# UCL/gp_emulator

Hardware: AMD Instinct MI355X
Metric: test-points/sec for predict(mean+var+grad), N_train=250 D=11 (higher is better)
Workload: dtype f64

## Files before the change

gp_emulator_amd/csrc/gp_abi.hip:

```cpp
#include "gp_predict_hip.h"

#include <hip/hip_runtime.h>

#include <cctype>
#include <chrono>
#include <cmath>
#include <cstdarg>
#include <cstdio>
#include <cstdlib>
#include <cstring>
#include <exception>
#include <memory>
#include <atomic>
#include <mutex>
#include <new>
#include <thread>
#include <type_traits>
#include <vector>

#include <sched.h>

#include "gp_dispatch.hpp"
#include "gp_generic_kernel.hpp"
#include "gp_hessian_kernel.hpp"
// ... 64 lines not shown
    hipError_t e_ = (expr);                                                           \
    if (e_ != hipSuccess)                                                             \
      return fail(GP_ERR_HIP, "%s failed: %s (%s:%d)", #expr, hipGetErrorString(e_),  \
                  __FILE__, __LINE__);                                                \
  } while (0)

struct gp_model {
  int device;
  int dtype;
  int n_train, n_inputs;
  int kernel_d, kernel_nb;
  int kernel_nk;
  int n_emulators;
  long long xa_stride, frags_stride, sd_stride;
  void* d_xa;
  void* d_frags;
  void* d_sd;
  std::vector<double> scale_host, centre_host;
  std::vector<double> xs_host;
  std::mutex h_mutex;
  void* d_pfrags;
  long long pfrags_stride;
};

constexpr int kPipeSlotsMax = 6;
static int pipe_slots() {
  static const int n = [] {
    const char* ev = getenv("GP_HOST_SLOTS");
    const int v = ev ? atoi(ev) : 3;
    return v < 2 ? 2 : (v > kPipeSlotsMax ? kPipeSlotsMax : v);
  }();
  return n;
}
#define kPipeSlots pipe_slots()
struct gp_pipe {
  bool ready = false;
  hipStream_t stream[kPipeSlotsMax] = {};
  hipEvent_t done[kPipeSlotsMax] = {};
  hipStream_t up = nullptr, down = nullptr;
  hipEvent_t in_there[kPipeSlotsMax] = {}, computed[kPipeSlotsMax] = {};
  void* stage_in[kPipeSlotsMax] = {};
  void* stage_out[kPipeSlotsMax] = {};
  void* dev[kPipeSlotsMax] = {};

  size_t stage_in_bytes = 0, stage_out_bytes = 0, dev_bytes = 0;
  std::unique_ptr<gph::ThreadPool> pool;
};

struct gp_cached_model {
  gp_model* model = nullptr;
  int host_dtype = 0, compute_dtype = 0, n_train = 0, n_inputs = 0, theta_size = 0;
  bool with_invq = false;
  std::vector<char> key;
  unsigned long long stamp = 0;
};
constexpr int kModelCacheSlots = 4;

static const int kTicketSlots = 256;

struct gp_ctx {
  int device;
  hipStream_t stream;
  int compute_units;
  void* scratch;
  size_t scratch_bytes;
  void* dbg;
  unsigned* tickets = nullptr;
  std::atomic<unsigned> ticket_next{0};
  gp_pipe pipe;
  gp_cached_model cache[kModelCacheSlots];
  unsigned long long cache_clock = 0;
};

struct gp_event {
  int device;
  hipEvent_t ev;
};

static const int kKernelD[] = {
#define GP_V(d) d,
    GP_FOR_EACH_KERNEL_D(GP_V)
#undef GP_V
};
static const int kKernelNK[] = {
#define GP_V(d) d,
    GP_FOR_EACH_KERNEL_NK(GP_V)
#undef GP_V
};

static int pick_kernel(int n_train, int n_inputs, int* kd, int* knb, int* knk = nullptr) {
  *kd = *knb = -1;
  int nk = -1;
  for (int d : kKernelD)
    if (d >= n_inputs) { *kd = d; break; }
  static const bool whole_blocks = [] {
    const char* ev = getenv("GP_NO_KSKIP");
    return ev && atoi(ev) != 0;
  }();
  const int need = (n_train + 3) / 4;
  for (int k : kKernelNK)
    if (k >= need && !(whole_blocks && k % 4 != 0)) { nk = k; break; }
  if (nk > 0) *knb = (nk + 3) / 4;
  if (knk) *knk = nk;
  if (*kd > 0 && *knb > 0) return GP_OK;
  if (n_train <= gpk::gkMaxN && n_inputs <= gpk::gkMaxD) {
    if (*kd < 0) *kd = n_inputs;
    *knb = 0;
    if (knk) *knk = 0;
    return GP_OK;
  }
  return fail(GP_ERR_UNSUPPORTED,
              "shape outside the compiled kernel set: n_train=%d (max %d), n_inputs=%d (max %d)",
              n_train, gpk::gkMaxN, n_inputs, gpk::gkMaxD);
}
static inline int rows_padded(int n_train, int knb) { return knb > 0 ? 16 * knb : 16 * ((n_train + 15) / 16); }
static inline int row_stride_of(int kd) { return gpk::row_stride(kd); }

template <typename T, typename TH = T>
static int pack_model(const TH* expX, const TH* inputs, const TH* invQt, const TH* invQ, int N,
                      int D, int theta_size, T* xa, T* frags, T* sd, T* b) {
  if (!expX || !inputs || !invQt || !xa || !sd || !b || (invQ && !frags))
    return fail(GP_ERR_INVALID, "null pointer");
  if (N <= 0 || D <= 0) return fail(GP_ERR_INVALID, "n_train and n_inputs must be positive");
  if (theta_size < D + 1)
    return fail(GP_ERR_INVALID, "theta_size=%d < n_inputs+1=%d", theta_size, D + 1);
  int kd, knb;
  int rc = pick_kernel(N, D, &kd, &knb);
  if (rc) return rc;
  const int DS = row_stride_of(kd);
  const int NP = rows_padded(N, knb);
  std::vector<double> sdd(kd, 0.0), ctr(kd, 0.0);
  for (int d = 0; d < D; ++d) {
    sdd[d] = std::sqrt((double)expX[d]);
    double sum = 0.0;
    for (int i = 0; i < N; ++i) sum += (double)inputs[(size_t)i * D + d];
    ctr[d] = (double)(T)(sum / N);
  }
  for (int d = 0; d < kd; ++d) {
    sd[d] = (T)sdd[d];
    sd[kd + d] = (T)ctr[d];
  }
  *b = (T)expX[D];
  sd[2 * kd] = (T)expX[D];
  const double lnb = std::log((double)expX[D]);
  std::memset(xa, 0, sizeof(T) * (size_t)NP * DS);
  for (int i = 0; i < N; ++i) {
    const size_t row = (size_t)(knb > 0 ? gpk::point_slot<T>(i) : i) * DS;
    double n2 = 0.0;
    for (int d = 0; d < D; ++d) {
      const T xr = (T)((double)sd[d] * ((double)inputs[(size_t)i * D + d] - ctr[d]));
      xa[row + d] = xr;
      n2 += (double)xr * (double)xr;
    }
    xa[row + kd] = (T)invQt[i];
    xa[row + kd + 1] = (T)(lnb - 0.5 * n2);
  }
  if (!invQ) return GP_OK;
  if (knb == 0) {
    for (size_t q = 0; q < (size_t)N * N; ++q) frags[q] = (T)invQ[q];
    return GP_OK;
  }
  const int nfp = gpk::frag_count_padded(knb, gpk::Geo<T>::kChunk);
  std::memset(frags, 0, sizeof(T) * (size_t)nfp * 64);
  for (int J = 0; J < knb; ++J)
    for (int I = J; I < knb; ++I)
      for (int s = 0; s < 4; ++s) {
        T* f = frags + (size_t)gpk::frag_index(I, J, s, knb) * 64;
        for (int l = 0; l < 64; ++l) {
          const int i = gpk::slot_point<T>(gpk::own_index<T>(I, s, l >> 4));
          const int j = gpk::slot_point<T>(16 * J + (l & 15));
          if (i >= N || j >= N) continue;
          double v = (double)invQ[(size_t)i * N + j];
          if (I > J) v += (double)invQ[(size_t)j * N + i];
          f[l] = (T)v;
        }
      }
  return GP_OK;
}

template <typename T>
static hipError_t launch(int knk, int kd, const gpk::PredictArgs<T>& a, int grid, bool var, hipStream_t s);
template <>
hipError_t launch<float>(int knk, int kd, const gpk::PredictArgs<float>& a, int grid, bool var, hipStream_t s) {
  switch (knk) {
#define GP_CASE(nk) \
  case nk: return var ? gpk::launch_predict_f32_##nk(kd, a, grid, s) : gpk::launch_mean_grad_f32_##nk(kd, a, grid, s);
    GP_FOR_EACH_KERNEL_NK(GP_CASE)
#undef GP_CASE
  }
  return hipErrorInvalidValue;
}
template <>
hipError_t launch<double>(int knk, int kd, const gpk::PredictArgs<double>& a, int grid, bool var, hipStream_t s) {
  switch (knk) {
#define GP_CASE(nk) \
  case nk: return var ? gpk::launch_predict_f64_##nk(kd, a, grid, s) : gpk::launch_mean_grad_f64_##nk(kd, a, grid, s);
    GP_FOR_EACH_KERNEL_NK(GP_CASE)
#undef GP_CASE
  }
  return hipErrorInvalidValue;
}

extern "C" {

const char* gp_last_error_string(void) { return g_err; }
const char* gp_version_string(void) { return "gp_predict_hip 0.1 (gfx950)"; }

int gp_device_count(int* count) {
  if (!count) return fail(GP_ERR_INVALID, "null pointer");
  int n = 0;
  hipError_t e = hipGetDeviceCount(&n);
  if (e != hipSuccess) {
    *count = 0;
    return fail(GP_ERR_NO_DEVICE, "hipGetDeviceCount: %s", hipGetErrorString(e));
  }
  *count = n;
  return GP_OK;
}

int gp_ctx_create(int device, gp_ctx** out) {
  if (!out) return fail(GP_ERR_INVALID, "null pointer");
  *out = nullptr;
  int n = 0;
  int rc = gp_device_count(&n);
  if (rc) return rc;
  if (n <= 0) return fail(GP_ERR_NO_DEVICE, "no HIP device visible");
  if (device < 0 || device >= n) return fail(GP_ERR_INVALID, "device %d out of range [0,%d)", device, n);
  HIP_TRY(hipSetDevice(device));
  hipDeviceProp_t prop;
  HIP_TRY(hipGetDeviceProperties(&prop, device));
  gp_ctx* c = new (std::nothrow) gp_ctx();
  if (!c) return fail(GP_ERR_NOMEM, "out of host memory");
  c->device = device;
  c->compute_units = prop.multiProcessorCount;
  c->scratch = nullptr;
  c->scratch_bytes = 0;
  c->dbg = nullptr;
  hipError_t e = hipStreamCreateWithFlags(&c->stream, hipStreamNonBlocking);
  if (e != hipSuccess) {
    delete c;
    return fail(GP_ERR_HIP, "hipStreamCreate: %s", hipGetErrorString(e));
  }
  e = hipMalloc((void**)&c->tickets, 4 * kTicketSlots * sizeof(unsigned));
  if (e == hipSuccess) e = hipMemset(c->tickets, 0, 4 * kTicketSlots * sizeof(unsigned));
  if (e != hipSuccess) {
    if (c->tickets) (void)hipFree(c->tickets);
    (void)hipStreamDestroy(c->stream);
    delete c;
    return fail(GP_ERR_HIP, "context item counters: %s", hipGetErrorString(e));
  }
  *out = c;
  return GP_OK;
}

int gp_ctx_destroy(gp_ctx* ctx) {
  if (!ctx) return GP_OK;
  (void)hipSetDevice(ctx->device);
  (void)hipStreamSynchronize(ctx->stream);
  for (auto& c : ctx->cache)
    if (c.model) gp_model_destroy(c.model);
  if (ctx->scratch) (void)hipFree(ctx->scratch);
  if (ctx->tickets) (void)hipFree(ctx->tickets);
  gp_pipe& pp = ctx->pipe;
  pp.pool.reset();
  for (int k = 0; k < kPipeSlots; ++k) {
    if (pp.stream[k]) (void)hipStreamSynchronize(pp.stream[k]);
    if (pp.stage_in[k]) (void)hipHostFree(pp.stage_in[k]);
    if (pp.stage_out[k]) (void)hipHostFree(pp.stage_out[k]);
    if (pp.dev[k]) (void)hipFree(pp.dev[k]);
    if (pp.done[k]) (void)hipEventDestroy(pp.done[k]);
    if (pp.in_there[k]) (void)hipEventDestroy(pp.in_there[k]);
    if (pp.computed[k]) (void)hipEventDestroy(pp.computed[k]);
    if (pp.stream[k]) (void)hipStreamDestroy(pp.stream[k]);
  }
  if (pp.up) { (void)hipStreamSynchronize(pp.up); (void)hipStreamDestroy(pp.up); }
  if (pp.down) { (void)hipStreamSynchronize(pp.down); (void)hipStreamDestroy(pp.down); }
  (void)hipStreamDestroy(ctx->stream);
  delete ctx;
  return GP_OK;
}

int gp_ctx_set_debug_buffer(gp_ctx* ctx, void* d_buffer) {
  if (!ctx) return fail(GP_ERR_INVALID, "null context");
  ctx->dbg = d_buffer;
  return GP_OK;
}

int gp_ctx_synchronize(gp_ctx* ctx) {
  if (!ctx) return fail(GP_ERR_INVALID, "null context");
  HIP_TRY(hipSetDevice(ctx->device));
  HIP_TRY(hipStreamSynchronize(ctx->stream));
  return GP_OK;
}

int gp_ctx_device_info(gp_ctx* ctx, int* compute_units, int64_t* hbm_bytes, char* name, int name_len) {
  if (!ctx) return fail(GP_ERR_INVALID, "null context");
  hipDeviceProp_t prop;
  HIP_TRY(hipGetDeviceProperties(&prop, ctx->device));
  if (compute_units) *compute_units = prop.multiProcessorCount;
  if (hbm_bytes) *hbm_bytes = (int64_t)prop.totalGlobalMem;
  if (name && name_len > 0) {
    snprintf(name, name_len, "%s (%s)", prop.name, prop.gcnArchName);
  }
  return GP_OK;
}

// ... 1780 lines not shown
```

gp_emulator_amd/csrc/gp_generic_kernel.hpp:

```cpp
#pragma once
#include "gp_predict_kernel.hpp"

namespace gpk {

constexpr int gkThreads = 256;
constexpr int gkMaxN = 1024;
constexpr int gkMaxD = 64;

template <typename T>
struct GenericArgs {
  const T* xa;
  const T* invQ;
  const T* sd;
  const T* testing;
  T* mu;
  T* var;
  T* deriv;
  long long M;
  int N, D;
  int ds, acol, dk;
  int deriv_row_major;
  int want_var;
};

template <typename T>
__device__ inline T row16_sum(T v) {
  v += __shfl_xor(v, 8, 64);
  v += __shfl_xor(v, 4, 64);
  v += __shfl_xor(v, 2, 64);
  v += __shfl_xor(v, 1, 64);
  return v;
}

template <typename T>
__global__ __launch_bounds__(gkThreads) void predict_generic_kernel(GenericArgs<T> p) {
  typedef Real<T> R;
  extern __shared__ __attribute__((aligned(16))) unsigned char g_raw[];
  T* s_k = reinterpret_cast<T*>(g_raw);
  const int ns = p.N + 1;
  T* s_t = s_k + 16 * ns;

  const int tid = threadIdx.x;
  const int ml = tid >> 4;
  const int jl = tid & 15;
  const T b = p.sd[2 * p.dk];
  const long long n_tiles = (p.M + 15) / 16;

  for (long long tile = blockIdx.x; tile < n_tiles; tile += gridDim.x) {
    const long long m = tile * 16 + ml;
    const long long mc = m < p.M ? m : p.M - 1;
    __syncthreads();
    for (int d = jl; d < p.D; d += 16)
      s_t[ml * p.D + d] = p.sd[d] * (p.testing[mc * p.D + d] - p.sd[p.dk + d]);
    __syncthreads();

    const T* t = &s_t[ml * p.D];
    T mu = T(0);
    for (int i = jl; i < p.N; i += 16) {
      const T* row = &p.xa[(long long)i * p.ds];
      T r2 = T(0);
      for (int d = 0; d < p.D; ++d) {
        const T dl = row[d] - t[d];
        r2 = fma(dl, dl, r2);
      }
      const T k = b * R::exp_(T(-0.5) * r2);
      s_k[ml * ns + i] = k;
      mu = fma(k, row[p.acol], mu);
    }
    mu = row16_sum(mu);
    if (jl == 0 && m < p.M) p.mu[m] = mu;

    for (int d = 0; d < p.D; ++d) {
      T gsum = T(0);
      for (int i = jl; i < p.N; i += 16) {
        const T* row = &p.xa[(long long)i * p.ds];
        gsum = fma(s_k[ml * ns + i] * row[p.acol], row[d] - t[d], gsum);
      }
      gsum = row16_sum(gsum) * p.sd[d];
      if (jl == 0 && m < p.M) {
        if (p.deriv_row_major) p.deriv[m * p.D + d] = gsum;
        else p.deriv[(long long)d * p.M + m] = gsum;
      }
    }
    if (!p.want_var) continue;
    __syncthreads();

    const T* kr = &s_k[ml * ns];
    T acc = T(0);
    for (int j = jl; j < p.N; j += 16) {
      T s = T(0);
      for (int i = 0; i < p.N; ++i) s = fma(p.invQ[(long long)i * p.N + j], kr[i], s);
      acc = fma(s, kr[j], acc);
    }
    acc = row16_sum(acc);
    if (jl == 0 && m < p.M) p.var[m] = b - acc;
  }
}

}
```

gp_emulator_amd/csrc/gp_hessian_kernel.hpp:

```cpp
#pragma once
#include "gp_predict_kernel.hpp"

#ifndef GP_HESS_ABLATE
#define GP_HESS_ABLATE 0
#endif

namespace gpk {

template <typename T>
struct HessianArgs {
  const T* xa;
  const T* sd;
  const T* testing;
  T* hess;
  long long M;
  int d_actual;
  int nb;
  int n_emulators;
  long long xa_stride, sd_stride, hess_stride;
};

constexpr int hkWaves = 4;
constexpr int hkThreads = hkWaves * 64;
constexpr int hkRowsPerWG = hkWaves * kTile;

__host__ __device__ constexpr int pairs_in_rows(int D, int lo, int hi) {
  int n = 0;
  for (int d = lo; d < hi; ++d) n += D - d;
  return n;
}
__host__ __device__ constexpr int split_row(int D) {
  int best = 0, bestdiff = 1 << 30;
  for (int r = 0; r <= D; ++r) {
    int a = pairs_in_rows(D, 0, r), b = pairs_in_rows(D, r, D);
    int diff = a > b ? a - b : b - a;
    if (diff < bestdiff) { bestdiff = diff; best = r; }
  }
  return best;
}

template <typename T, int D, int LO, int HI>
__device__ __forceinline__ void hessian_pass(const T* s_xa, const T* s_sd, const T (&t)[D], T b,
                                             int nb, int g, bool row_ok, int d_actual, T* out) {
  typedef Real<T> R;
  constexpr int DS = row_stride(D);
  constexpr int NP_ = pairs_in_rows(D, LO, HI);
  T acc[NP_];
#pragma unroll
  for (int q = 0; q < NP_; ++q) acc[q] = T(0);
  T mu = T(0);
  T nxt[D + 1];
  {
    const T* row = &s_xa[R::own_sub(0, g) * DS];
#pragma unroll
    for (int d = 0; d <= D; ++d) nxt[d] = row[d];
  }
#pragma unroll 1
  for (int qq = 0; qq < 4 * nb; ++qq) {
    T dl[D];
    T r2p[4] = {T(0), T(0), T(0), T(0)};
#pragma unroll
    for (int d = 0; d < D; ++d) {
      dl[d] = nxt[d] - t[d];
      r2p[d & 3] = fma(dl[d], dl[d], r2p[d & 3]);
    }
    const T alpha = nxt[D];
    {
      const int qn = (qq + 1 < 4 * nb) ? qq + 1 : 0;
      const T* row = &s_xa[(16 * (qn >> 2) + R::own_sub(qn & 3, g)) * DS];
#pragma unroll
      for (int d = 0; d <= D; ++d) nxt[d] = row[d];
    }
    const T r2 = (r2p[0] + r2p[1]) + (r2p[2] + r2p[3]);
    const T w = b * R::exp_(T(-0.5) * r2) * alpha;
    mu += w;
    int q = 0;
#pragma unroll
    for (int d = LO; d < HI; ++d) {
      const T wd = w * dl[d];
#pragma unroll
      for (int d2 = d; d2 < D; ++d2) {
        acc[q] = fma(wd, dl[d2], acc[q]);
        ++q;
      }
    }
  }
#if GP_HESS_ABLATE == 2
  T keep = mu;
#pragma unroll
  for (int q = 0; q < NP_; ++q) keep += acc[q];
  if (keep == T(-12345.678)) out[0] = keep;
  return;
#endif
  mu = xor_reduce_groups(mu);
  int q = 0;
#pragma unroll
  for (int d = LO; d < HI; ++d) {
#pragma unroll
    for (int d2 = d; d2 < D; ++d2) {
      T v = xor_reduce_groups(acc[q]) * (s_sd[d] * s_sd[d2]);
      if (d2 == d) v = fma(-(s_sd[d] * s_sd[d]), mu, v);
      ++q;
#if GP_HESS_ABLATE == 1
      if (v == T(-12345.678)) out[0] = v;
#else
      if (row_ok && d < d_actual && d2 < d_actual) {
        if ((d & 3) == g) out[d * d_actual + d2] = v;
        if (d2 != d && (d2 & 3) == g) out[d2 * d_actual + d] = v;
      }
#endif
    }
  }
}

template <typename T, int D, bool BATCH = false>
__global__ __launch_bounds__(hkThreads, 2) void hessian_kernel(HessianArgs<T> p) {
  typedef Real<T> R;
  constexpr int DS = row_stride(D);
  constexpr int NPAIR = D * (D + 1) / 2;
  constexpr int kSplit = (NPAIR * (int)sizeof(T) / 4 > 144) ? split_row(D) : 0;
  extern __shared__ __attribute__((aligned(16))) unsigned char s_raw[];
  T* s_xa = reinterpret_cast<T*>(s_raw);

  const int tid = threadIdx.x;
  const int lane = tid & 63;
  const int wave = __builtin_amdgcn_readfirstlane(tid >> 6);
  const int ml = lane & 15;
  const int g = lane >> 4;
  const int np = 16 * p.nb;

  T* s_sd = s_xa + np * DS;
  const long long n_groups = (p.M + hkRowsPerWG - 1) / hkRowsPerWG;
  const long long n_items = BATCH ? n_groups * p.n_emulators : n_groups;
  T b;
  auto load_emulator = [&](int e_) __attribute__((always_inline)) {
    const T* xa_ = p.xa;
    const T* sd_ = p.sd;
    if constexpr (BATCH) {
      xa_ += (long long)e_ * p.xa_stride;
      sd_ += (long long)e_ * p.sd_stride;
    }
    for (int i = tid; i < np * DS; i += hkThreads) s_xa[i] = xa_[i];
    if (tid < 2 * D) s_sd[tid] = ((tid % D) < p.d_actual) ? sd_[tid] : T(0);
    b = sd_[2 * D];
  };
  int cur_e = BATCH ? (int)(blockIdx.x / n_groups) : 0;
  load_emulator(cur_e);
  __syncthreads();

  for (long long item = blockIdx.x; item < n_items; item += gridDim.x) {
    long long grp = item;
    T* hess_e = p.hess;
    if constexpr (BATCH) {
      const int e = (int)(item / n_groups);
      grp = item - e * n_groups;
      hess_e += (long long)e * p.hess_stride;
      if (e != cur_e) {
        cur_e = e;
        __syncthreads();
        load_emulator(e);
        __syncthreads();
      }
    }
    const long long m = grp * hkRowsPerWG + wave * kTile + ml;
    const long long mc = m < p.M ? m : p.M - 1;
    T t[D];
#pragma unroll
    for (int d = 0; d < D; ++d)
      t[d] = (d < p.d_actual) ? s_sd[d] * (p.testing[mc * p.d_actual + d] - s_sd[D + d]) : T(0);
    T* out = hess_e + mc * (long long)p.d_actual * p.d_actual;
    const bool row_ok = m < p.M;
    if constexpr (kSplit > 0) {
      hessian_pass<T, D, 0, kSplit>(s_xa, s_sd, t, b, p.nb, g, row_ok, p.d_actual, out);
      hessian_pass<T, D, kSplit, D>(s_xa, s_sd, t, b, p.nb, g, row_ok, p.d_actual, out);
    } else {
      hessian_pass<T, D, 0, D>(s_xa, s_sd, t, b, p.nb, g, row_ok, p.d_actual, out);
    }
  }
}

}
```

gp_emulator_amd/csrc/gp_predict_few_kernel.hpp:

```cpp
#pragma once
#include "gp_predict_kernel.hpp"

namespace gpk {

constexpr int fkWaves = 8;
constexpr int fkThreads = fkWaves * 64;
constexpr int fkMaxKSteps = 4 * 20;

template <typename T, int D, bool kVar = true>
__global__ __launch_bounds__(fkThreads, 2) void predict_few_kernel(PredictArgs<T> p, int NB) {
  typedef Real<T> R;
  typedef typename R::acc_t acc_t;
  constexpr int DS = row_stride(D);
  constexpr int kVals = D + 2;

  __shared__ __attribute__((aligned(16))) T s_xa[4 * fkMaxKSteps * row_stride(D)];
  __shared__ T s_k[kVar ? fkMaxKSteps : 1][64];
  __shared__ T s_part[fkWaves][kTile][kVals];

  const int tid = threadIdx.x;
  const int lane = tid & 63;
  const int w = __builtin_amdgcn_readfirstlane(tid >> 6);
  const int ml = lane & 15, g = lane >> 4;
  const int n_tiles = (int)((p.M + kTile - 1) / kTile);
  const int e = blockIdx.x / n_tiles, tile = blockIdx.x - e * n_tiles;
  const int NKS = 4 * NB;

  const T* xa = p.xa + e * p.xa_stride;
  const T* frags = p.frags + e * p.frags_stride;
  (void)frags;
  const T* sdp = p.sd + e * p.sd_stride;
  const long long m = (long long)tile * kTile + ml;
  const long long mc = m < p.M ? m : p.M - 1;

  {
    const int n = 16 * NB * DS;
#pragma unroll 4
    for (int i = tid; i < n; i += fkThreads) s_xa[i] = xa[i];
  }

  T t[D];
  T gm = T(0);
#pragma unroll
  for (int d = 0; d < D; ++d) {
    const bool live = d < p.d_actual;
    const int dc = live ? d : p.d_actual - 1;
    const T sc = !live ? T(0) : p.rows_prescaled ? T(1) : sdp[d];
    const T ce = (!live || p.rows_prescaled) ? T(0) : sdp[D + d];
    t[d] = sc * (p.testing[mc * p.d_actual + dc] - ce);
    gm = fma(t[d], t[d], gm);
  }
  gm *= T(-0.5);
  const T poison = gm - gm;
  const T b = sdp[2 * D];
  __syncthreads();

  T mu = T(0);
  T ga[D];
#pragma unroll
  for (int d = 0; d < D; ++d) ga[d] = T(0);
#pragma unroll 1
  for (int ks = w; ks < NKS; ks += fkWaves) {
    const int i = own_index<T>(ks >> 2, ks & 3, g);
    const T* row = &s_xa[i * DS];
    T x[D];
#pragma unroll
    for (int d = 0; d < D; ++d) x[d] = row[d];
    const T al = row[D];
    T k;
    if constexpr (R::kExpand) {
      k = row[D + 1] + gm;
#pragma unroll
      for (int d = 0; d < D; ++d) k = fma(x[d], t[d], k);
      k = R::exp_(k);
    } else {
      T r2 = T(0);
#pragma unroll
      for (int d = 0; d < D; ++d) {
        x[d] -= t[d];
        r2 = fma(x[d], x[d], r2);
      }
      k = b * R::exp_(T(-0.5) * r2);
    }
    if constexpr (kVar) s_k[ks][lane] = k;
    const T wgt = k * al;
    mu += wgt;
#pragma unroll
    for (int d = 0; d < D; ++d) ga[d] = fma(wgt, x[d], ga[d]);
  }
  mu = xor_reduce_groups(mu);
  xor_reduce_groups_n<T, D>(ga);
  if (g == 0) {
    s_part[w][ml][0] = mu;
#pragma unroll
    for (int d = 0; d < D; ++d) s_part[w][ml][1 + d] = ga[d];
  }
  __syncthreads();

  if constexpr (kVar) {
  T vacc = T(0);
  auto column_block = [&](const int J) __attribute__((always_inline)) {
    const T* f = frags + ((size_t)frag_index(J, J, 0, NB) * 64 + lane);
    const int n = 4 * (NB - J);
    acc_t acc = acc_t{T(0), T(0), T(0), T(0)};
    T a_cur[4], a_nxt[4];
#pragma unroll
    for (int s = 0; s < 4; ++s) a_cur[s] = f[(size_t)s * 64];
#pragma unroll 1
    for (int q = 0; q < n; q += 4) {
      const int qn = q + 4 < n ? q + 4 : q;
#pragma unroll
      for (int s = 0; s < 4; ++s) a_nxt[s] = f[(size_t)(qn + s) * 64];
#pragma unroll
      for (int s = 0; s < 4; ++s) acc = R::mfma(a_cur[s], s_k[4 * J + q + s][lane], acc);
#pragma unroll
      for (int s = 0; s < 4; ++s) a_cur[s] = a_nxt[s];
    }
#pragma unroll
    for (int r = 0; r < 4; ++r) vacc = fma(acc[r], s_k[4 * J + r][lane], vacc);
  };
  for (int pr = w; 2 * pr < NB; pr += fkWaves) {
    column_block(pr);
    if (NB - 1 - pr != pr) column_block(NB - 1 - pr);
  }
  vacc = xor_reduce_groups(vacc);
  if (g == 0) s_part[w][ml][1 + D] = vacc;
  __syncthreads();
  }

  if (w == 0 && m < p.M) {
    auto total = [&](const int v) __attribute__((always_inline)) {
      T s = s_part[0][ml][v];
#pragma unroll
      for (int k = 1; k < fkWaves; ++k) s += s_part[k][ml][v];
      return s;
    };
    const T mean = total(0) + poison;
    T* o_mu = p.mu + e * p.M;
    T* o_der = p.deriv + e * p.M * p.d_actual;
    if (g == 0) o_mu[m] = mean;
    if constexpr (kVar) {
      if (g == 1) p.var[e * p.M + m] = b - total(1 + D) + poison;
    }
#pragma unroll
    for (int d = 0; d < D; ++d) {
      if ((d & 3) == g && d < p.d_actual) {
        const T gsum = total(1 + d);
        const T gd = sdp[d] * (R::kExpand ? fma(-t[d], mean, gsum) : gsum + poison);
        if (p.deriv_row_major) o_der[m * p.d_actual + d] = gd;
        else o_der[(long long)d * p.M + m] = gd;
      }
    }
  }
}

}
```

gp_emulator_amd/csrc/gp_predict_kernel.hpp:

```cpp
#pragma once
#include <hip/hip_runtime.h>
#include <stdint.h>
#include <type_traits>
#include <utility>

namespace gpk {

#ifndef GP_WAVES
#define GP_WAVES 8
#endif
#ifndef GP_WAVES_F32
#define GP_WAVES_F32 12
#endif
#ifndef GP_CHUNK
#define GP_CHUNK 64
#endif
#ifndef GP_CHUNK_F32
#define GP_CHUNK_F32 192
#endif
#ifndef GP_ABLATE
#define GP_ABLATE 0
#endif
#ifndef GP_AHEAD
#define GP_AHEAD 4
#endif
#ifndef GP_AHEAD_F32
#define GP_AHEAD_F32 8
#endif
#ifndef GP_RING_PIN
#define GP_RING_PIN 1
#endif
#ifndef GP_MU_DOUBLE
#define GP_MU_DOUBLE 1
#endif
#ifndef GP_ESTRIN
#define GP_ESTRIN 0
#endif
#ifndef GP_DOTSPLIT
#define GP_DOTSPLIT 1
#endif
#ifndef GP_GROUP_F64
#define GP_GROUP_F64 1
#endif
#ifndef GP_STAMPS
#define GP_STAMPS 0
#endif
constexpr int kTile = 16;
template <typename T, bool kVar = true> struct Geo {
  static constexpr int kWaves = sizeof(T) == 8 ? GP_WAVES : GP_WAVES_F32;
  static constexpr int kThreads = kWaves * 64;
#ifndef GP_WG_PER_CU_SMALL
#define GP_WG_PER_CU_SMALL 0
#endif
  static constexpr int kWGPerCU = kWaves >= 8 ? 1 : (GP_WG_PER_CU_SMALL > 0 ? GP_WG_PER_CU_SMALL : 8 / kWaves);
  static constexpr int kWavesPerSimd = kWaves >= 8 ? kWaves / 4 : kWGPerCU * kWaves / 4;
  static constexpr int kRowsPerWG = kWaves * kTile;
  static constexpr int kChunk = sizeof(T) == 8 ? GP_CHUNK : GP_CHUNK_F32;
};
#ifndef GP_MG_WAVES
#define GP_MG_WAVES 12
#endif
#ifndef GP_MG_WAVES_F32
#define GP_MG_WAVES_F32 16
#endif
#ifndef GP_MG_WG_PER_CU
#define GP_MG_WG_PER_CU 1
#endif
template <typename T> struct Geo<T, false> {
  static constexpr int kWaves = sizeof(T) == 8 ? GP_MG_WAVES : GP_MG_WAVES_F32;
  static constexpr int kThreads = kWaves * 64;
  static constexpr int kWGPerCU = GP_MG_WG_PER_CU;
  static constexpr int kWavesPerSimd = kWGPerCU * kWaves / 4;
  static constexpr int kRowsPerWG = kWaves * kTile;
  static constexpr int kChunk = 1;
};

typedef double f64x4 __attribute__((ext_vector_type(4)));
typedef float f32x4 __attribute__((ext_vector_type(4)));

template <typename F, int... Is>
__device__ __forceinline__ void static_for_impl(F&& f, std::integer_sequence<int, Is...>) {
  (f(std::integral_constant<int, Is>{}), ...);
}
template <int N, typename F>
__device__ __forceinline__ void static_for(F&& f) {
  static_for_impl(f, std::make_integer_sequence<int, N>{});
}

template <typename T> struct Real;
template <> struct Real<double> {
  typedef f64x4 acc_t;
  static constexpr bool kExpand = true;
  static constexpr int kGroup = GP_GROUP_F64;
  __host__ __device__ static constexpr int own_sub(int r, int g) { return 4 * r + g; }
  __device__ static inline acc_t mfma(double a, double b, acc_t c) {
    return __builtin_amdgcn_mfma_f64_16x16x4f64(a, b, c, 0, 0, 0);
  }
  __device__ static inline double exp_(double x) {
    x = __builtin_fmax(x, -1000.0);
    const double n = __builtin_rint(x * 1.4426950408889634);
    double r = fma(n, -6.93147180559945286e-01, x);
    r = fma(n, -2.31904681384629956e-17, r);
#if GP_ESTRIN
    const double r2 = r * r;
    const double p01 = fma(1.00000000000000666e+00, r, 1.0);
    const double p23 = fma(1.66666666665544028e-01, r, 5.00000000000000555e-01);
    const double p45 = fma(8.33333338566834801e-03, r, 4.16666666665732183e-02);
    const double p67 = fma(1.98411702695461072e-04, r, 1.38888889324666632e-03);
    const double p89 = fma(2.76401812311866076e-06, r, 2.48015043709117912e-05);
    const double r4 = r2 * r2;
    const double q0 = fma(r2, p23, p01);
    const double q1 = fma(r2, p67, p45);
    const double q2 = fma(r2, 2.76263485910095559e-07, p89);
    const double r8 = r4 * r4;
    const double s0 = fma(r4, q1, q0);
    const double p = fma(r8, q2, s0);
#else
    double p = 2.76263485910095559e-07;
    p = fma(p, r, 2.76401812311866076e-06);
    p = fma(p, r, 2.48015043709117912e-05);
    p = fma(p, r, 1.98411702695461072e-04);
    p = fma(p, r, 1.38888889324666632e-03);
    p = fma(p, r, 8.33333338566834801e-03);
    p = fma(p, r, 4.16666666665732183e-02);
    p = fma(p, r, 1.66666666665544028e-01);
    p = fma(p, r, 5.00000000000000555e-01);
    p = fma(p, r, 1.00000000000000666e+00);
    p = fma(p, r, 1.0);
#endif
    return ldexp(p, (int)n);
  }
  template <int GP>
  __device__ static inline void exp_n(double (&x)[GP]) {
    double n[GP], r[GP], p[GP];
#pragma unroll
    for (int u = 0; u < GP; ++u) x[u] = __builtin_fmax(x[u], -1000.0);
#pragma unroll
    for (int u = 0; u < GP; ++u) n[u] = __builtin_rint(x[u] * 1.4426950408889634);
#pragma unroll
    for (int u = 0; u < GP; ++u) r[u] = fma(n[u], -6.93147180559945286e-01, x[u]);
#pragma unroll
    for (int u = 0; u < GP; ++u) r[u] = fma(n[u], -2.31904681384629956e-17, r[u]);
#pragma unroll
    for (int u = 0; u < GP; ++u) p[u] = 2.76263485910095559e-07;
    constexpr double c[10] = {2.76401812311866076e-06, 2.48015043709117912e-05, 1.98411702695461072e-04,
                              1.38888889324666632e-03, 8.33333338566834801e-03, 4.16666666665732183e-02,
                              1.66666666665544028e-01, 5.00000000000000555e-01, 1.00000000000000666e+00, 1.0};
#pragma unroll
    for (int j = 0; j < 10; ++j) {
#pragma unroll
      for (int u = 0; u < GP; ++u) p[u] = fma(p[u], r[u], c[j]);
    }
#pragma unroll
    for (int u = 0; u < GP; ++u) x[u] = ldexp(p[u], (int)n[u]);
  }
};
template <> struct Real<float> {
  typedef f32x4 acc_t;
  static constexpr bool kExpand = false;
#ifndef GP_GROUP_F32
#define GP_GROUP_F32 2
#endif
  static constexpr int kGroup = GP_GROUP_F32;
  __host__ __device__ static constexpr int own_sub(int r, int g) { return 4 * g + r; }
  __device__ static inline acc_t mfma(float a, float b, acc_t c) {
    return __builtin_amdgcn_mfma_f32_16x16x4f32(a, b, c, 0, 0, 0);
  }
  __device__ static inline float exp_(float x) { return __expf(x); }
  template <int GP>
  __device__ static inline void exp_n(float (&x)[GP]) {
#pragma unroll
    for (int u = 0; u < GP; ++u) x[u] = __expf(x[u]);
  }
};

template <typename T>
__host__ __device__ constexpr int own_index(int I, int s, int g) {
  return 16 * I + Real<T>::own_sub(s, g);
}

template <typename T>
__host__ __device__ constexpr int point_slot(int n) {
  return 16 * (n / 16) + Real<T>::own_sub((n % 16) / 4, n % 4);
}
template <typename T>
__host__ __device__ constexpr int slot_point(int slot) {
  for (int q = 0; q < 16; ++q)
    if (Real<T>::own_sub(q / 4, q % 4) == slot % 16) return 16 * (slot / 16) + q;
  return -1;
}

struct FragId { int I, J, s; };
__host__ __device__ constexpr int frag_count(int NB) { return NB * (NB + 1) / 2 * 4; }
__host__ __device__ constexpr int frag_col_offset(int J, int NB) { return J * NB - J * (J - 1) / 2; }
__host__ __device__ constexpr FragId frag_at(int n, int NB) {
  const int pair = n >> 2;
  int J = 0;
  while (J + 1 < NB && frag_col_offset(J + 1, NB) <= pair) ++J;
  return FragId{J + pair - frag_col_offset(J, NB), J, n & 3};
}
__host__ __device__ constexpr int frag_index(int I, int J, int s, int NB) {
  return (frag_col_offset(J, NB) + (I - J)) * 4 + s;
}
__host__ __device__ constexpr int frag_count_padded(int NB, int chunk) {
  return (frag_count(NB) + chunk - 1) / chunk * chunk;
}

__host__ __device__ constexpr int row_stride(int D) { return (D + 2 + 3) & ~3; }
#ifndef GP_XA_PAD
#define GP_XA_PAD 1
#endif
template <typename T> __host__ __device__ constexpr int xa_lds_stride(int D) {
  return (GP_XA_PAD && sizeof(T) == 4 && row_stride(D) % 16 == 0) ? row_stride(D) + 4 : row_stride(D);
}

#ifndef GP_FRAG_BUFS
#define GP_FRAG_BUFS 3
#endif
#ifndef GP_FRAG_BUFS_F32
#define GP_FRAG_BUFS_F32 2
#endif
constexpr int kLdsBudget = 160 * 1024;
constexpr int kLdsSlack = 32;
template <typename T>
__host__ __device__ constexpr int predict_lds_bytes(int D, int NK, int bufs) {
  const int NP = 16 * ((NK + 3) / 4);
  return (int)sizeof(T) * (NP * xa_lds_stride<T>(D) + bufs * Geo<T>::kChunk * 64 + (2 * D + 1) + 2 * D +
                           2 * Geo<T>::kWaves * kTile * D) + kLdsSlack;
}
template <typename T>
__host__ __device__ constexpr int frag_buffers(int D, int NK) {
  const int want = sizeof(T) == 8 ? GP_FRAG_BUFS : GP_FRAG_BUFS_F32;
  return want > 2 && predict_lds_bytes<T>(D, NK, want) <= kLdsBudget ? want : 2;
}

template <typename T>
struct PredictArgs {
  const T* xa;
  const T* frags;
  const T* sd;
  const T* testing;
  T* mu;
  T* var;
  T* deriv;
  long long M;
  int d_actual;
  int deriv_row_major;
  int n_emulators;
  long long xa_stride, frags_stride, sd_stride;
  unsigned long long* dbg;
  int rows_prescaled;
};

template <int XOR>
__device__ __forceinline__ unsigned swap_halves(unsigned x, unsigned& other) {
  if constexpr (XOR == 16) {
    auto r = __builtin_amdgcn_permlane16_swap(x, x, false, false);
    other = r[1];
    return r[0];
  } else {
    auto r = __builtin_amdgcn_permlane32_swap(x, x, false, false);
    other = r[1];
    return r[0];
  }
}
template <int XOR>
__device__ __forceinline__ float pair_sum(float v) {
  unsigned o, a = swap_halves<XOR>(__float_as_uint(v), o);
  return __uint_as_float(a) + __uint_as_float(o);
}
template <int XOR>
__device__ __forceinline__ double pair_sum(double v) {
  const unsigned long long u = (unsigned long long)__double_as_longlong(v);
  unsigned lo_o, hi_o;
  const unsigned lo_a = swap_halves<XOR>((unsigned)u, lo_o);
  const unsigned hi_a = swap_halves<XOR>((unsigned)(u >> 32), hi_o);
  const double a = __longlong_as_double((long long)(((unsigned long long)hi_a << 32) | lo_a));
  const double o = __longlong_as_double((long long)(((unsigned long long)hi_o << 32) | lo_o));
  return a + o;
}

template <typename T, int N>
__device__ inline void xor_reduce_groups_n(T* v) {
#pragma unroll
  for (int i = 0; i < N; ++i) v[i] = pair_sum<32>(pair_sum<16>(v[i]));
}

template <typename T>
__device__ inline T xor_reduce_groups(T v) {
  return pair_sum<32>(pair_sum<16>(v));
}

template <typename T, int kWaves = Geo<T>::kWaves, int kChunk = Geo<T>::kChunk>
__device__ __forceinline__ void stage_chunk(const T* src, T* dst, int wave, int lane) {
  constexpr int kBytes = kChunk * 64 * (int)sizeof(T);
  constexpr int kPieces = kBytes / 1024;
  static_assert(kPieces * 1024 == kBytes, "chunk must be whole 1 KiB pieces");
  const unsigned voff = (unsigned)lane * 16u;
  const unsigned lds0 = (unsigned)(uintptr_t)(
      (__attribute__((address_space(3))) char*)(reinterpret_cast<char*>(dst)));
#pragma unroll
  for (int pc0 = 0; pc0 < kPieces; pc0 += kWaves) {
    const int pc = pc0 + wave;
    if (pc0 + kWaves <= kPieces || pc < kPieces) {
      const char* s = reinterpret_cast<const char*>(src) + pc * 1024;
      const unsigned m0v = __builtin_amdgcn_readfirstlane(lds0 + pc * 1024);
      unsigned keep;
      asm volatile(
          "s_mov_b32 %0, m0\n\t"
          "s_mov_b32 m0, %1\n\t"
          "s_nop 4\n\t"
          "global_load_lds_dwordx4 %2, %3\n\t"
          "s_mov_b32 m0, %0"
          : "=&s"(keep)
          : "s"(m0v), "v"(voff), "s"(s)
          : "memory");
    }
  }
}
template <typename T, int NP>
__device__ __forceinline__ void stage_pieces(const T* src, T* dst, int first_piece, int lane) {
  const unsigned voff = (unsigned)lane * 16u;
  const unsigned lds0 = (unsigned)(uintptr_t)(
      (__attribute__((address_space(3))) char*)(reinterpret_cast<char*>(dst)));
#pragma unroll
  for (int i = 0; i < NP; ++i) {
    const int pc = first_piece + i;
    const char* s = reinterpret_cast<const char*>(src) + pc * 1024;
    const unsigned m0v = __builtin_amdgcn_readfirstlane(lds0 + pc * 1024);
    unsigned keep;
    asm volatile(
        "s_mov_b32 %0, m0\n\t"
        "s_mov_b32 m0, %1\n\t"
        "s_nop 4\n\t"
        "global_load_lds_dwordx4 %2, %3\n\t"
        "s_mov_b32 m0, %0"
        : "=&s"(keep)
        : "s"(m0v), "v"(voff), "s"(s)
        : "memory");
  }
}
__device__ __forceinline__ void dma_wait() { asm volatile("s_waitcnt vmcnt(0)" ::: "memory"); }

#if GP_STAMPS == 1
#define GP_STAMP(seg)                                                                    \
  do {                                                                                   \
    __builtin_amdgcn_sched_barrier(0);                                                   \
    unsigned long long now_;                                                             \
    asm volatile("s_memtime %0\n\ts_waitcnt lgkmcnt(0)" : "=s"(now_)::"memory");         \
    __builtin_amdgcn_sched_barrier(0);                                                   \
    seg_sum[seg] += now_ - seg_t0;                                                       \
    seg_t0 = now_;                                                                       \
  } while (0)
#else
#define GP_STAMP(seg) do { } while (0)
#endif

template <typename T, int D, int NK, bool kVar = true>
__global__ __launch_bounds__((Geo<T, kVar>::kThreads), (Geo<T, kVar>::kWavesPerSimd)) void predict_kernel(PredictArgs<T> p) {
  typedef Real<T> R;
  typedef Geo<T, kVar> G;
  constexpr int kThreads = G::kThreads;
  constexpr int kRowsPerWG = G::kRowsPerWG;
  typedef typename R::acc_t acc_t;
  constexpr int NB = (NK + 3) / 4;
  constexpr int KL = NK - 4 * (NB - 1);
  constexpr int NP = 16 * NB;
  constexpr int DSG = row_stride(D);
  constexpr int DS = xa_lds_stride<T>(D);
  constexpr int NF = frag_count(NB);
  constexpr int kChunk = G::kChunk;
  constexpr int NCH = (NF + kChunk - 1) / kChunk;
  constexpr int kBufs = kVar ? frag_buffers<T>(D, NK) : 1;
  constexpr int kLook = kBufs - 2;

  __shared__ __attribute__((aligned(16))) T s_xa[NP * DS];
  __shared__ __attribute__((aligned(16))) T s_fr[kBufs][kVar ? kChunk * 64 : 1];
  __shared__ T s_sd[2 * D + 1];
  __shared__ T s_ts[2 * D];
  __shared__ T s_rows[2][G::kWaves][kTile * D];
  static_assert(!kVar || (int)(sizeof(s_xa) + sizeof(s_fr) + sizeof(s_sd) + sizeof(s_ts) + sizeof(s_rows)) + kLdsSlack ==
                             predict_lds_bytes<T>(D, NK, kBufs), "predict_lds_bytes() does not count the kernel's LDS arrays");

  const int tid = threadIdx.x;
  const int lane = tid & 63;
  const int wave = __builtin_amdgcn_readfirstlane(tid >> 6);
  const int ml = lane & 15;
  const int g = lane >> 4;

  const int n_groups = (int)((p.M + kRowsPerWG - 1) / kRowsPerWG);
  int e = 0, cur_e = -1;
  int grp = blockIdx.x;
  while (grp >= n_groups && e < p.n_emulators) { grp -= n_groups; ++e; }

  constexpr int NJ = (kTile * D + 63) / 64;
  auto fetch_rows = [&](int grp_, T (&regs)[NJ]) {
    const long long e0 = ((long long)grp_ * kRowsPerWG + wave * kTile) * p.d_actual;
    const long long emax = p.M * p.d_actual - 1;
#pragma unroll
    for (int j = 0; j < NJ; ++j) {
      long long e_ = e0 + lane + 64 * j;
      e_ = e_ < emax ? e_ : emax;
      regs[j] = p.testing[e_];
    }
  };
  auto stash_rows = [&](int buf_, const T (&regs)[NJ]) {
#pragma unroll
    for (int j = 0; j < NJ; ++j) asm volatile("" ::"v"(regs[j]));
#pragma unroll
    for (int j = 0; j < NJ; ++j)
      if (lane + 64 * j < kTile * p.d_actual) s_rows[buf_][wave][lane + 64 * j] = regs[j];
  };
  int rbuf = 0;
  T rregs[NJ];
  if (e < p.n_emulators) {
    fetch_rows(grp, rregs);
    stash_rows(0, rregs);
  }
#if GP_STAMPS
  unsigned long long seg_sum[8] = {0, 0, 0, 0, 0, 0, 0, 0};
  unsigned long long seg_t0;
  asm volatile("s_memtime %0\n\ts_waitcnt lgkmcnt(0)" : "=s"(seg_t0)::"memory");
#endif

  for (; e < p.n_emulators;) {
    if (e != cur_e) {
      cur_e = e;
      __syncthreads();
      const T* xa = p.xa + e * p.xa_stride;
      for (int i = tid; i < NP * DSG; i += kThreads) s_xa[(i / DSG) * DS + i % DSG] = xa[i];
      const T* sdp = p.sd + e * p.sd_stride;
      if (tid < 2 * D + 1) {
        const bool live = tid == 2 * D || (tid % D) < p.d_actual;
        s_sd[tid] = live ? sdp[tid] : T(0);
        if (tid < 2 * D)
          s_ts[tid] = !live ? T(0) : !p.rows_prescaled ? sdp[tid] : tid < D ? T(1) : T(0);
      }
      if constexpr (!kVar) __syncthreads();
    }
    const T* frags = p.frags + e * p.frags_stride;
    T* o_mu = p.mu + e * p.M;
    T* o_der = p.deriv + e * p.M * p.d_actual;
    const long long m = (long long)grp * kRowsPerWG + wave * kTile + ml;
    const long long mc = m < p.M ? m : p.M - 1;

    if constexpr (kVar) {
      __syncthreads();
      static_for<1 + kLook>([&](auto cc) {
        constexpr int c = decltype(cc)::value;
        if constexpr (c < NCH) stage_chunk<T, G::kWaves, kChunk>(frags + c * kChunk * 64, &s_fr[c][0], wave, lane);
      });
    } else {
      (void)frags;
      __builtin_amdgcn_fence(__ATOMIC_ACQ_REL, "wavefront");
      __builtin_amdgcn_wave_barrier();
    }
    const T b = s_sd[2 * D];
    GP_STAMP(0);

    T t[D];
    T gm = T(0);
    {
      T sdv[D], cv[D], rv[D];
#pragma unroll
      for (int d = 0; d < D; ++d) {
        const int dc = d < p.d_actual ? d : p.d_actual - 1;
        sdv[d] = s_ts[d];
        cv[d] = s_ts[D + d];
        rv[d] = s_rows[rbuf][wave][ml * p.d_actual + dc];
      }
#pragma unroll
      for (int d = 0; d < D; ++d) {
        t[d] = sdv[d] * (rv[d] - cv[d]);
        gm = fma(t[d], t[d], gm);
      }
    }
    gm *= T(-0.5);
    const T poison = gm - gm;

    asm volatile("" :: "v"(gm));
    int e_next = e, grp_next = grp + gridDim.x;
    while (grp_next >= n_groups && e_next < p.n_emulators) { grp_next -= n_groups; ++e_next; }
    fetch_rows(e_next < p.n_emulators ? grp_next : grp, rregs);

    GP_STAMP(1);
    T kv[NK];
#if GP_MU_DOUBLE
    double mu = 0.0;
#else
    T mu = T(0);
#endif
    T ga[D];
#pragma unroll
    for (int d = 0; d < D; ++d) ga[d] = T(0);

    constexpr int GP = R::kGroup;
    static_for<(NK + GP - 1) / GP>([&](auto qc) {
      constexpr int q0 = decltype(qc)::value * GP;
      constexpr int GU = NK - q0 < GP ? NK - q0 : GP;
      T x[GP][D];
      T al[GP];
      T k[GP];
#pragma unroll
      for (int u = 0; u < GU; ++u) {
        const int q = q0 + u;
        const int i = own_index<T>(q >> 2, q & 3, g);
        const T* row = &s_xa[i * DS];
#pragma unroll
        for (int d = 0; d < D; ++d) x[u][d] = row[d];
        al[u] = row[D];
        if constexpr (R::kExpand) k[u] = row[D + 1] + gm;
      }
#pragma unroll
      for (int u = 0; u < GU; ++u) {
#if GP_ABLATE == 2
        continue;
#endif
        if constexpr (R::kExpand) {
          T part[GP_DOTSPLIT];
          part[0] = k[u];
#pragma unroll
          for (int c = 1; c < GP_DOTSPLIT; ++c) part[c] = T(0);
#pragma unroll
          for (int d = 0; d < D; ++d) part[d % GP_DOTSPLIT] = fma(x[u][d], t[d], part[d % GP_DOTSPLIT]);
#pragma unroll
          for (int c = 1; c < GP_DOTSPLIT; ++c) part[0] += part[c];
          k[u] = part[0];
        } else {
          T r2 = T(0);
#pragma unroll
          for (int d = 0; d < D; ++d) {
            x[u][d] -= t[d];
            r2 = fma(x[u][d], x[u][d], r2);
          }
          k[u] = T(-0.5) * r2;
        }
      }
#pragma unroll
      for (int u = 0; u < GU; ++u) {
#if GP_ABLATE == 2
        k[u] = x[u][0] + t[0];
#else
        k[u] = R::kExpand ? R::exp_(k[u]) : b * R::exp_(k[u]);
#endif
        if constexpr (kVar) kv[q0 + u] = k[u];
      }
#pragma unroll
      for (int u = 0; u < GU; ++u) {
        const T w = k[u] * al[u];
        mu += (decltype(mu))w;
#if GP_ABLATE == 2
        ga[u % D] += w;
#else
#pragma unroll
        for (int d = 0; d < D; ++d) ga[d] = fma(w, x[u][d], ga[d]);
#endif
      }
    });
    GP_STAMP(2);
    const T mu_t = (T)xor_reduce_groups(mu) + poison;
    static_for<(D + 5) / 6>([&](auto bc) {
      constexpr int d0 = decltype(bc)::value * 6;
      constexpr int nb_ = (D - d0 < 6) ? (D - d0) : 6;
      xor_reduce_groups_n<T, nb_>(&ga[d0]);
    });
    {
      T sdv[D];
#pragma unroll
      for (int d = 0; d < D; ++d) sdv[d] = s_sd[d];
#pragma unroll
      for (int d = 0; d < D; ++d)
        ga[d] = sdv[d] * (R::kExpand ? fma(-t[d], mu_t, ga[d]) : ga[d]);
    }

    if (m < p.M) {
      if (g == 0) o_mu[m] = mu_t;
      int gs = g;
      asm volatile("" : "+v"(gs));
      T gq[(D + 3) / 4];
#pragma unroll
      for (int q = 0; q < (D + 3) / 4; ++q) {
        gq[q] = ga[4 * q];
#pragma unroll
        for (int u = 1; u < 4; ++u)
          if (4 * q + u < D) gq[q] = gs == u ? ga[4 * q + u] : gq[q];
      }
      if (p.deriv_row_major) {
        T* o_row = o_der + m * p.d_actual + gs;
#pragma unroll
        for (int q = 0; q < (D + 3) / 4; ++q)
          if (4 * q + gs < p.d_actual) o_row[4 * q] = gq[q];
      } else {
        T* o_row = o_der + gs * p.M + m;
#pragma unroll
        for (int q = 0; q < (D + 3) / 4; ++q)
          if (4 * q + gs < p.d_actual) o_row[4 * q * p.M] = gq[q];
      }
    }

    GP_STAMP(3);
    stash_rows(rbuf ^ 1, rregs);
    if constexpr (!kVar) {
      rbuf ^= 1;
      e = e_next;
      grp = grp_next;
      continue;
    } else {

    T* o_var = p.var + e * p.M;
    T vacc = T(0);
    acc_t acc;
    constexpr int kAhead = sizeof(T) == 4 ? GP_AHEAD_F32 : GP_AHEAD;
    T afr[kAhead];
#if GP_ABLATE == 1
    static_for<NK>([&](auto qc) { vacc += kv[decltype(qc)::value]; });
    static_for<0>([&](auto fc) {
#else
    static_for<NF>([&](auto fc) {
#endif
      constexpr int f = decltype(fc)::value;
      constexpr int c = f / kChunk, fl = f % kChunk;
      constexpr FragId fid = frag_at(f, NB);
      constexpr int I = fid.I, J = fid.J, s = fid.s;
      if constexpr (fl == 0) {
#if GP_ABLATE == 4
        if constexpr (c == 0) { dma_wait(); __syncthreads(); }
#else
        if constexpr (c == 0 || c + kLook < NCH) {
          dma_wait();
          if constexpr (kLook > 0) {
            if constexpr (c > 0) __builtin_amdgcn_sched_barrier(0);
            asm volatile("s_barrier" ::: "memory");
            if constexpr (c > 0) __builtin_amdgcn_sched_barrier(0);
          } else {
            __syncthreads();
          }
          if constexpr (c + kLook + 1 < NCH)
            stage_chunk<T, G::kWaves, kChunk>(frags + (c + kLook + 1) * kChunk * 64,
                                              &s_fr[(c + kLook + 1) % kBufs][0], wave, lane);
        }
#endif
        static_for<kAhead - 1>([&](auto jc) {
          constexpr int n = f + decltype(jc)::value;
          if constexpr (n < NF && (c == 0 || n / kChunk > c - 1 + kLook)) {
#if GP_ABLATE >= 3
            afr[n % kAhead] = kv[n % NK];
#else
            afr[n % kAhead] = s_fr[(n / kChunk) % kBufs][(n % kChunk) * 64 + lane];
#endif
          }
        });
      }
      {
        constexpr int n = f + kAhead - 1;
        if constexpr (n < NF && n / kChunk <= c + kLook) {
#if GP_ABLATE >= 3
          afr[n % kAhead] = kv[(f + 1) % NK];
#else
          afr[n % kAhead] = s_fr[(n / kChunk) % kBufs][(n % kChunk) * 64 + lane];
#endif
        }
      }
      if constexpr (I == J && s == 0) acc = acc_t{T(0), T(0), T(0), T(0)};
      if constexpr (4 * I + s < NK) acc = R::mfma(afr[f % kAhead], kv[4 * I + s], acc);
#if GP_RING_PIN
      if constexpr (sizeof(T) == 4 || GP_RING_PIN > 1) __builtin_amdgcn_sched_barrier(0);
#endif
      if constexpr (I == NB - 1 && s == 3) {
#pragma unroll
        for (int r = 0; r < (J == NB - 1 ? KL : 4); ++r) vacc = fma(acc[r], kv[4 * J + r], vacc);
      }
    });
    rbuf ^= 1;
    GP_STAMP(4);
    vacc = xor_reduce_groups(vacc);
    if (m < p.M && g == 1) o_var[m] = b - vacc + poison;

    e = e_next;
    grp = grp_next;
    GP_STAMP(5);
    }
  }
#if GP_STAMPS
  if (lane == 0 && p.dbg) {
    for (int k_ = 0; k_ < 8; ++k_) atomicAdd(&p.dbg[k_], seg_sum[k_]);
    atomicAdd(&p.dbg[7], 1ull);
  }
#endif
}

}
```

Baseline: 757.0 million.

## Fuse exp range reduction via magic-add rounding and prefetch next tile's fragments across seam

Replaces the rint-plus-convert range reduction in the f64 exp with a single FMA against a rounding magic constant, taking the integer exponent from the low bits. The clamp moves to a separate exp_clamped used by the generic, hessian and few kernels, while the fused kernel instead zeroes out far-away test points and rejects training points beyond a reach limit on the host. The main predict kernel also gains a 'seam' schedule: the first two chunks of inverse-covariance fragments for the next tile are staged during the last chunks of the current tile, rather than after a barrier at the start of the next iteration. This is meant to hide the ring-buffer refill latency and some ALU work, at the cost of extra barriers and more complex sync.

Result: faster. 768.5 million (median of 6 runs) (+1.5%).

```diff
diff --git a/gp_emulator_amd/csrc/gp_abi.hip b/gp_emulator_amd/csrc/gp_abi.hip
--- a/gp_emulator_amd/csrc/gp_abi.hip
+++ b/gp_emulator_amd/csrc/gp_abi.hip
@@ -240,6 +240,10 @@
       xa[row + d] = xr;
       n2 += (double)xr * (double)xr;
     }
+    if (sizeof(T) == 8 && knb > 0 && 0.5 * n2 > gpk::Real<double>::kMaxHalfNorm2)
+      return fail(GP_ERR_UNSUPPORTED,
+                  "training point %d lies %.4g length scales from the training mean (the fused kernel takes up to %.0f)",
+                  i, std::sqrt(n2), std::sqrt(2.0 * gpk::Real<double>::kMaxHalfNorm2));
     xa[row + kd] = (T)invQt[i];
     xa[row + kd + 1] = (T)(lnb - 0.5 * n2);
   }
diff --git a/gp_emulator_amd/csrc/gp_generic_kernel.hpp b/gp_emulator_amd/csrc/gp_generic_kernel.hpp
--- a/gp_emulator_amd/csrc/gp_generic_kernel.hpp
+++ b/gp_emulator_amd/csrc/gp_generic_kernel.hpp
@@ -63,7 +63,7 @@
         const T dl = row[d] - t[d];
         r2 = fma(dl, dl, r2);
       }
-      const T k = b * R::exp_(T(-0.5) * r2);
+      const T k = b * R::exp_clamped(T(-0.5) * r2);
       s_k[ml * ns + i] = k;
       mu = fma(k, row[p.acol], mu);
     }
diff --git a/gp_emulator_amd/csrc/gp_hessian_kernel.hpp b/gp_emulator_amd/csrc/gp_hessian_kernel.hpp
--- a/gp_emulator_amd/csrc/gp_hessian_kernel.hpp
+++ b/gp_emulator_amd/csrc/gp_hessian_kernel.hpp
@@ -72,7 +72,7 @@
       for (int d = 0; d <= D; ++d) nxt[d] = row[d];
     }
     const T r2 = (r2p[0] + r2p[1]) + (r2p[2] + r2p[3]);
-    const T w = b * R::exp_(T(-0.5) * r2) * alpha;
+    const T w = b * R::exp_clamped(T(-0.5) * r2) * alpha;
     mu += w;
     int q = 0;
 #pragma unroll
diff --git a/gp_emulator_amd/csrc/gp_predict_few_kernel.hpp b/gp_emulator_amd/csrc/gp_predict_few_kernel.hpp
--- a/gp_emulator_amd/csrc/gp_predict_few_kernel.hpp
+++ b/gp_emulator_amd/csrc/gp_predict_few_kernel.hpp
@@ -72,7 +72,7 @@
       k = row[D + 1] + gm;
 #pragma unroll
       for (int d = 0; d < D; ++d) k = fma(x[d], t[d], k);
-      k = R::exp_(k);
+      k = R::exp_clamped(k);
     } else {
       T r2 = T(0);
 #pragma unroll
@@ -80,7 +80,7 @@
         x[d] -= t[d];
         r2 = fma(x[d], x[d], r2);
       }
-      k = b * R::exp_(T(-0.5) * r2);
+      k = b * R::exp_clamped(T(-0.5) * r2);
     }
     if constexpr (kVar) s_k[ks][lane] = k;
     const T wgt = k * al;
diff --git a/gp_emulator_amd/csrc/gp_predict_kernel.hpp b/gp_emulator_amd/csrc/gp_predict_kernel.hpp
--- a/gp_emulator_amd/csrc/gp_predict_kernel.hpp
+++ b/gp_emulator_amd/csrc/gp_predict_kernel.hpp
@@ -35,6 +35,9 @@
 #endif
 #ifndef GP_ESTRIN
 #define GP_ESTRIN 0
+#endif
+#ifndef GP_EXP_FUSED
+#define GP_EXP_FUSED 1
 #endif
 #ifndef GP_DOTSPLIT
 #define GP_DOTSPLIT 1
@@ -96,9 +99,17 @@
   __device__ static inline acc_t mfma(double a, double b, acc_t c) {
     return __builtin_amdgcn_mfma_f64_16x16x4f64(a, b, c, 0, 0, 0);
   }
-  __device__ static inline double exp_(double x) {
+  static constexpr double kRoundMagic = 6755399441055744.0;
+  __host__ __device__ static inline double exp_(double x) {
+#if GP_EXP_FUSED
+    const double s = fma(x, 1.4426950408889634, kRoundMagic);
+    const double n = s - kRoundMagic;
+    const int ni = (int)(unsigned)__builtin_bit_cast(unsigned long long, s);
+#else
     x = __builtin_fmax(x, -1000.0);
     const double n = __builtin_rint(x * 1.4426950408889634);
+    const int ni = (int)n;
+#endif
     double r = fma(n, -6.93147180559945286e-01, x);
     r = fma(n, -2.31904681384629956e-17, r);
 #if GP_ESTRIN
@@ -128,15 +139,30 @@
     p = fma(p, r, 1.00000000000000666e+00);
     p = fma(p, r, 1.0);
 #endif
-    return ldexp(p, (int)n);
-  }
+    return ldexp(p, ni);
+  }
+  __host__ __device__ static inline double exp_clamped(double x) { return exp_(__builtin_fmax(x, -1000.0)); }
   template <int GP>
   __device__ static inline void exp_n(double (&x)[GP]) {
     double n[GP], r[GP], p[GP];
+    int ni[GP];
 #pragma unroll
     for (int u = 0; u < GP; ++u) x[u] = __builtin_fmax(x[u], -1000.0);
-#pragma unroll
-    for (int u = 0; u < GP; ++u) n[u] = __builtin_rint(x[u] * 1.4426950408889634);
+#if GP_EXP_FUSED
+#pragma unroll
+    for (int u = 0; u < GP; ++u) r[u] = fma(x[u], 1.4426950408889634, kRoundMagic);
+#pragma unroll
+    for (int u = 0; u < GP; ++u) {
+      n[u] = r[u] - kRoundMagic;
+      ni[u] = (int)(unsigned)__builtin_bit_cast(unsigned long long, r[u]);
+    }
+#else
+#pragma unroll
+    for (int u = 0; u < GP; ++u) {
+      n[u] = __builtin_rint(x[u] * 1.4426950408889634);
+      ni[u] = (int)n[u];
+    }
+#endif
 #pragma unroll
     for (int u = 0; u < GP; ++u) r[u] = fma(n[u], -6.93147180559945286e-01, x[u]);
 #pragma unroll
@@ -152,8 +178,10 @@
       for (int u = 0; u < GP; ++u) p[u] = fma(p[u], r[u], c[j]);
     }
 #pragma unroll
-    for (int u = 0; u < GP; ++u) x[u] = ldexp(p[u], (int)n[u]);
-  }
+    for (int u = 0; u < GP; ++u) x[u] = ldexp(p[u], ni[u]);
+  }
+  static constexpr double kMaxHalfNorm2 = 67108864.0;
+  static constexpr double kFarG = 134217728.0;
 };
 template <> struct Real<float> {
   typedef f32x4 acc_t;
@@ -167,6 +195,7 @@
     return __builtin_amdgcn_mfma_f32_16x16x4f32(a, b, c, 0, 0, 0);
   }
   __device__ static inline float exp_(float x) { return __expf(x); }
+  __device__ static inline float exp_clamped(float x) { return __expf(x); }
   template <int GP>
   __device__ static inline void exp_n(float (&x)[GP]) {
 #pragma unroll
@@ -219,6 +248,9 @@
 #endif
 #ifndef GP_FRAG_BUFS_F32
 #define GP_FRAG_BUFS_F32 2
+#endif
+#ifndef GP_SEAM
+#define GP_SEAM 2
 #endif
 constexpr int kLdsBudget = 160 * 1024;
 constexpr int kLdsSlack = 32;
@@ -373,6 +405,11 @@
   constexpr int NCH = (NF + kChunk - 1) / kChunk;
   constexpr int kBufs = kVar ? frag_buffers<T>(D, NK) : 1;
   constexpr int kLook = kBufs - 2;
+  constexpr bool kSeamOk = kVar && kBufs == 3 && NCH >= 3 && NCH % 3 == 0;
+  constexpr bool kSeamAblated = (GP_ABLATE == 5 || GP_ABLATE == 6) && kSeamOk;
+  constexpr bool kSeam = GP_SEAM && !kSeamAblated && kSeamOk;
+  constexpr bool kSeamTop = kSeam || kSeamAblated;
+  constexpr bool kSeamAlways = kSeam && GP_SEAM == 2;
 
   __shared__ __attribute__((aligned(16))) T s_xa[NP * DS];
   __shared__ __attribute__((aligned(16))) T s_fr[kBufs][kVar ? kChunk * 64 : 1];
@@ -424,8 +461,17 @@
 #endif
 
   for (; e < p.n_emulators;) {
+    const T* frags = p.frags + e * p.frags_stride;
+    auto open_ring = [&]() {
+      __syncthreads();
+      static_for<1 + kLook>([&](auto cc) {
+        constexpr int c = decltype(cc)::value;
+        if constexpr (c < NCH) stage_chunk<T, G::kWaves, kChunk>(frags + c * kChunk * 64, &s_fr[c][0], wave, lane);
+      });
+    };
     if (e != cur_e) {
       cur_e = e;
+      if constexpr (kSeamAlways) dma_wait();
       __syncthreads();
       const T* xa = p.xa + e * p.xa_stride;
       for (int i = tid; i < NP * DSG; i += kThreads) s_xa[(i / DSG) * DS + i % DSG] = xa[i];
@@ -437,19 +483,15 @@
           s_ts[tid] = !live ? T(0) : !p.rows_prescaled ? sdp[tid] : tid < D ? T(1) : T(0);
       }
       if constexpr (!kVar) __syncthreads();
-    }
-    const T* frags = p.frags + e * p.frags_stride;
+      if constexpr (kVar && kSeamTop) open_ring();
+    }
     T* o_mu = p.mu + e * p.M;
     T* o_der = p.deriv + e * p.M * p.d_actual;
     const long long m = (long long)grp * kRowsPerWG + wave * kTile + ml;
     const long long mc = m < p.M ? m : p.M - 1;
 
     if constexpr (kVar) {
-      __syncthreads();
-      static_for<1 + kLook>([&](auto cc) {
-        constexpr int c = decltype(cc)::value;
-        if constexpr (c < NCH) stage_chunk<T, G::kWaves, kChunk>(frags + c * kChunk * 64, &s_fr[c][0], wave, lane);
-      });
+      if constexpr (!kSeamTop) open_ring();
     } else {
       (void)frags;
       __builtin_amdgcn_fence(__ATOMIC_ACQ_REL, "wavefront");
@@ -477,11 +519,18 @@
     }
     gm *= T(-0.5);
     const T poison = gm - gm;
+    if constexpr (R::kExpand && GP_EXP_FUSED) {
+      const bool in_reach = gm >= T(-R::kFarG);
+#pragma unroll
+      for (int d = 0; d < D; ++d) t[d] = in_reach ? t[d] : T(0);
+      gm = in_reach ? gm : T(-R::kFarG);
+    }
 
     asm volatile("" :: "v"(gm));
     int e_next = e, grp_next = grp + gridDim.x;
     while (grp_next >= n_groups && e_next < p.n_emulators) { grp_next -= n_groups; ++e_next; }
     fetch_rows(e_next < p.n_emulators ? grp_next : grp, rregs);
+    const bool ahead = kSeam && e_next == e;
 
     GP_STAMP(1);
     T kv[NK];
@@ -570,7 +619,7 @@
       for (int d = 0; d < D; ++d) sdv[d] = s_sd[d];
 #pragma unroll
       for (int d = 0; d < D; ++d)
-        ga[d] = sdv[d] * (R::kExpand ? fma(-t[d], mu_t, ga[d]) : ga[d]);
+        ga[d] = R::kExpand ? sdv[d] * fma(-t[d], mu_t, ga[d]) : fma(sdv[d], ga[d], poison);
     }
 
     if (m < p.M) {
@@ -635,9 +684,23 @@
           } else {
             __syncthreads();
           }
-          if constexpr (c + kLook + 1 < NCH)
+          if constexpr (c + kLook + 1 < NCH) {
             stage_chunk<T, G::kWaves, kChunk>(frags + (c + kLook + 1) * kChunk * 64,
                                               &s_fr[(c + kLook + 1) % kBufs][0], wave, lane);
+          } else if constexpr (kSeam && c == NCH - 2) {
+            if (kSeamAlways || ahead) stage_chunk<T, G::kWaves, kChunk>(frags, &s_fr[0][0], wave, lane);
+          }
+        } else if constexpr (GP_ABLATE == 6 && kSeamAblated && c == NCH - 1) {
+          __builtin_amdgcn_sched_barrier(0);
+          asm volatile("s_barrier" ::: "memory");
+          __builtin_amdgcn_sched_barrier(0);
+        } else if constexpr (kSeam && c == NCH - 1) {
+          if (kSeamAlways || ahead) {
+            __builtin_amdgcn_sched_barrier(0);
+            asm volatile("s_barrier" ::: "memory");
+            __builtin_amdgcn_sched_barrier(0);
+            stage_chunk<T, G::kWaves, kChunk>(frags + kChunk * 64, &s_fr[1][0], wave, lane);
+          }
         }
 #endif
         static_for<kAhead - 1>([&](auto jc) {
@@ -681,6 +744,7 @@
     GP_STAMP(5);
     }
   }
+  if constexpr (kSeamAlways) dma_wait();
 #if GP_STAMPS
   if (lane == 0 && p.dbg) {
     for (int k_ = 0; k_ < 8; ++k_) atomicAdd(&p.dbg[k_], seg_sum[k_]);
```
